# ai4ce/V2X-Sim

Measured on AMD Instinct MI355X. Metric: BEV frames/sec, V2VNet 5-agent detection (256x256 BEV), higher is better.
Workload: dtype bf16

## Files before the change

v2x-sim_amd/csrc/conv_halo.hip:

```cpp
#include "common.h"
#include <cstdlib>

static __device__ __attribute__((aligned(64))) unsigned int g_zero_page_h[16];

typedef const __attribute__((address_space(1))) void *gptr_t;
typedef __attribute__((address_space(3))) void *lptr_t;

__device__ __forceinline__ void glds16h(const void *g, char *lds_wave_base) {
    __builtin_amdgcn_global_load_lds((gptr_t)g, (lptr_t)lds_wave_base, 16, 0, 0);
}

struct HaloArgs {
    const uint16_t *in0;
    const uint16_t *in1;
    const uint32_t *bits;
    int zbits;
    int N, H, W;
    const uint16_t *w;
    const float *scale, *shift;
    int relu;
    void *out;
    int out_cstride, out_coff;
    const uint16_t *w2;
    const float *scale2, *shift2;
// ... 554 lines not shown
    const int fj = lane & 15, fq = lane >> 4;
    char *pb = s_patch + grp * PATCH_BYTES;

    for (int off = wave * 1024; off < W_BYTES; off += 8192)
        glds16h(reinterpret_cast<const char *>(a.w) + off + lane * 16, s_w + off);

    constexpr bool TABLES = (COUT2 == 0);
    constexpr int NP1 = (NS1 + 255) / 256, NP0 = (NS0 + 255) / 256;
    int tb1[TABLES ? NP1 : 1], tb0[NP0 ? NP0 : 1];
#pragma unroll
    for (int t = 0; t < (TABLES ? NP1 : 0); ++t) {
        const int L = wv * 64 + t * 256 + lane;
        const int pix = L / SPP1, phys = L - pix * SPP1;
        const int pr = pix / PW, pc = pix - pr * PW;
        tb1[t] = pix < PH * PW ? (((pr * a.W + pc) * C1 + swz<SPP1>(phys, pc) * 8) | (pr << 20) | (pc << 24)) : -1;
    }
    if constexpr (C0 > 0) {
        constexpr int S0 = SPP0 ? SPP0 : 1;
#pragma unroll
        for (int t = 0; t < NP0; ++t) {
            const int L = wv * 64 + t * 256 + lane;
            const int pix = L / S0, phys = L - pix * S0;
            const int pr = pix / PW0, pc = pix - pr * PW0;
            tb0[t] = pix < PH0 * PW0 ? (((pr * (a.W >> 1) + pc) * C0 + swz<(SPP0 ? SPP0 : 4)>(phys, pc) * 8) | (pr << 20) | (pc << 24)) : -1;
        }
    }

    const int txy = a.tiles_x * a.tiles_y;
    auto coords = [&](int tile, int &n, int &y0, int &x0) {
        n = tile / txy;
        const int r = tile - n * txy;
        const int ty = r / a.tiles_x;
        y0 = ty * TH;
        x0 = (r - ty * a.tiles_x) * TW;
    };
    auto load_patch = [&](int tile) {
        int n, y0, x0;
        coords(tile, n, y0, x0);
        if constexpr (TABLES) {
            const unsigned base = ((unsigned)(n * a.H + y0 - 1) * (unsigned)a.W + (unsigned)(x0 - 1)) * (unsigned)C1;
#pragma unroll
            for (int t = 0; t < NP1; ++t) {
                if (wv * 64 + t * 256 >= NS1) break;
                const int y = y0 - 1 + ((tb1[t] >> 20) & 15), x = x0 - 1 + ((tb1[t] >> 24) & 63);
                const bool ok = tb1[t] >= 0 && (unsigned)y < (unsigned)a.H && (unsigned)x < (unsigned)a.W;
                glds16h(ok ? (const void *)(a.in1 + (base + (unsigned)(tb1[t] & 0xfffff))) : (const void *)g_zero_page_h,
                        pb + NS0 * 16 + (wv * 64 + t * 256) * 16);
            }
        } else {
            for (int base = wv * 64; base < NS1; base += 256) {
                const int L = base + lane;
                const int pix = L / SPP1, phys = L - pix * SPP1;
                const int pr = pix / PW, pc = pix - pr * PW;
                const int y = y0 - 1 + pr, x = x0 - 1 + pc;
                const bool ok = pix < PH * PW && (unsigned)y < (unsigned)a.H && (unsigned)x < (unsigned)a.W;
                const unsigned off = ((unsigned)(n * a.H + y) * (unsigned)a.W + (unsigned)x) * (unsigned)C1 + swz<SPP1>(phys, pc) * 8;
                glds16h(ok ? (const void *)(a.in1 + off) : (const void *)g_zero_page_h, pb + NS0 * 16 + base * 16);
            }
        }
        if constexpr (C0 > 0) {
            const int Hs = a.H >> 1, Ws = a.W >> 1;
            const unsigned base = ((unsigned)(n * Hs + (y0 >> 1) - 1) * (unsigned)Ws + (unsigned)((x0 >> 1) - 1)) * (unsigned)C0;
#pragma unroll
            for (int t = 0; t < NP0; ++t) {
                if (wv * 64 + t * 256 >= NS0) break;
                const int y = (y0 >> 1) - 1 + ((tb0[t] >> 20) & 15), x = (x0 >> 1) - 1 + ((tb0[t] >> 24) & 63);
                const bool ok = tb0[t] >= 0 && (unsigned)y < (unsigned)Hs && (unsigned)x < (unsigned)Ws;
                glds16h(ok ? (const void *)(a.in0 + (base + (unsigned)(tb0[t] & 0xfffff))) : (const void *)g_zero_page_h,
                        pb + (wv * 64 + t * 256) * 16);
            }
        }
    };

    f32x4_t acc[TCO][4];
    constexpr int KC0 = C0 / 32, KC1 = C1 / 32, KC = KC0 + KC1, NG = 3 * KC;
    struct Frags {
        bf16x8_t A[3][TCO];
        bf16x8_t B[8];
    };
    auto load_group = [&](int g, Frags &F) {
        const int kx = g / KC, kk = g - kx * KC;
        if (kk < KC0) {
#pragma unroll
            for (int ky = 0; ky < 3; ++ky) {
                const int kslot = (ky * 3 + kx) * (SPP0 + SPP1) + kk * 4 + fq;
#pragma unroll
                for (int i = 0; i < TCO; ++i)
                    F.A[ky][i] = *reinterpret_cast<const bf16x8_t *>(s_w + (kslot * COUT + i * 16 + fj) * 16);
            }
#pragma unroll
            for (int hr = 0; hr < 3; ++hr)
#pragma unroll
                for (int ch = 0; ch < 2; ++ch) {
                    const int pr = wv + hr;
                    const int pc = ((ch * 16 + fj + kx - 1) >> 1) + 1;
                    F.B[hr * 2 + ch] = *reinterpret_cast<const bf16x8_t *>(pb + ((pr * PW0 + pc) * (SPP0 ? SPP0 : 1) + swz<(SPP0 ? SPP0 : 4)>(kk * 4 + fq, pc)) * 16);
                }
        } else {
            const int kc = kk - KC0;
#pragma unroll
            for (int ky = 0; ky < 3; ++ky) {
                const int kslot = (ky * 3 + kx) * (SPP0 + SPP1) + SPP0 + kc * 4 + fq;
#pragma unroll
                for (int i = 0; i < TCO; ++i)
                    F.A[ky][i] = *reinterpret_cast<const bf16x8_t *>(s_w + (kslot * COUT + i * 16 + fj) * 16);
            }
#pragma unroll
            for (int rr = 0; rr < 4; ++rr)
#pragma unroll
                for (int ch = 0; ch < 2; ++ch) {
                    const int pr = 2 * wv + rr;
                    const int pc = ch * 16 + fj + kx;
                    F.B[rr * 2 + ch] = *reinterpret_cast<const bf16x8_t *>(pb + NS0 * 16 + ((pr * PW + pc) * SPP1 + swz<SPP1>(kc * 4 + fq, pc)) * 16);
                }
        }
    };
    auto mma_group = [&](int g, const Frags &F) {
        const bool half = (g % KC) < KC0;
#pragma unroll
        for (int ky = 0; ky < 3; ++ky)
#pragma unroll
            for (int i = 0; i < TCO; ++i)
#pragma unroll
                for (int f = 0; f < 4; ++f) {
                    const int r = f >> 1, ch = f & 1;
                    const int row = half ? (((r + ky - 1) >> 1) + 1) : (r + ky);
                    acc[i][f] = __builtin_amdgcn_mfma_f32_16x16x32_bf16(F.A[ky][i], F.B[row * 2 + ch], acc[i][f], 0, 0, 0);
                }
    };
    auto compute = [&]() {
#pragma unroll
        for (int i = 0; i < TCO; ++i)
#pragma unroll
            for (int f = 0; f < 4; ++f) acc[i][f] = (f32x4_t){0.f, 0.f, 0.f, 0.f};
        if constexpr (TCO == 2) {
            Frags fr[2];
            load_group(0, fr[0]);
#pragma unroll
            for (int g = 0; g < NG; ++g) {
                if (g + 1 < NG) load_group(g + 1, fr[(g + 1) & 1]);
                __builtin_amdgcn_sched_barrier(0);
                mma_group(g, fr[g & 1]);
                __builtin_amdgcn_sched_barrier(0);
            }
        } else {
            static_assert(C0 == 0 || TCO == 2, "the 64-channel form has one full-resolution source");
            bf16x8_t B[8], A[2][TCO];
            auto load_A = [&](int g, int ky, bf16x8_t (&Ak)[TCO]) {
                const int kx = g / KC, kc = g - kx * KC;
                const int kslot = (ky * 3 + kx) * (SPP0 + SPP1) + SPP0 + kc * 4 + fq;
#pragma unroll
                for (int i = 0; i < TCO; ++i) Ak[i] = *reinterpret_cast<const bf16x8_t *>(s_w + (kslot * COUT + i * 16 + fj) * 16);
            };
#pragma unroll
            for (int g = 0; g < NG; ++g) {
                const int kx = g / KC, kc = g - kx * KC;
#pragma unroll
                for (int rr = 0; rr < 4; ++rr)
#pragma unroll
                    for (int ch = 0; ch < 2; ++ch) {
                        const int pr = 2 * wv + rr, pc = ch * 16 + fj + kx;
                        B[rr * 2 + ch] = *reinterpret_cast<const bf16x8_t *>(pb + NS0 * 16 + ((pr * PW + pc) * SPP1 + swz<SPP1>(kc * 4 + fq, pc)) * 16);
                    }
                load_A(g, 0, A[0]);
#pragma unroll
                for (int ky = 0; ky < 3; ++ky) {
                    if (ky < 2) load_A(g, ky + 1, A[(ky + 1) & 1]);
                    __builtin_amdgcn_sched_barrier(0);
#pragma unroll
                    for (int i = 0; i < TCO; ++i)
#pragma unroll
                        for (int f = 0; f < 4; ++f)
                            acc[i][f] = __builtin_amdgcn_mfma_f32_16x16x32_bf16(A[ky & 1][i], B[((f >> 1) + ky) * 2 + (f & 1)], acc[i][f], 0, 0, 0);
                    __builtin_amdgcn_sched_barrier(0);
                }
            }
        }
    };
    auto epilogue = [&](int tile) {
        int n, y0, x0;
        coords(tile, n, y0, x0);
        int zo = 0;
        asm volatile("" : "+v"(zo));
        const float *ss = s_ss + zo;
        if constexpr (COUT2 > 0) {
            bf16x8_t w2f[TCO2][COUT / 32];
            int w2off = fj * COUT + fq * 8;
            asm volatile("" : "+v"(w2off));
#pragma unroll
            for (int i2 = 0; i2 < TCO2; ++i2)
#pragma unroll
                for (int ks = 0; ks < COUT / 32; ++ks)
                    w2f[i2][ks] = *reinterpret_cast<const bf16x8_t *>(a.w2 + w2off + i2 * 16 * COUT + ks * 32);
            asm volatile("s_waitcnt vmcnt(0)" ::: "memory");
#pragma unroll
            for (int f = 0; f < 4; ++f) {
                bf16x8_t hb[COUT / 32];
#pragma unroll
                for (int ks = 0; ks < COUT / 32; ++ks) {
                    float h[8];
#pragma unroll
                    for (int hf = 0; hf < 2; ++hf) {
                        const int i = 2 * ks + hf;
                        const int kappa = 32 * (i >> 1) + 8 * fq + 4 * (i & 1);
                        const float4 sc = *reinterpret_cast<const float4 *>(ss + kappa);
                        const float4 sf = *reinterpret_cast<const float4 *>(ss + COUT + kappa);
                        h[hf * 4 + 0] = acc[i][f][0] * sc.x + sf.x;
                        h[hf * 4 + 1] = acc[i][f][1] * sc.y + sf.y;
                        h[hf * 4 + 2] = acc[i][f][2] * sc.z + sf.z;
                        h[hf * 4 + 3] = acc[i][f][3] * sc.w + sf.w;
                    }
                    uint4 p;
                    p.x = pack_bf16x2(h[0], h[1]);
                    p.y = pack_bf16x2(h[2], h[3]);
                    p.z = pack_bf16x2(h[4], h[5]);
                    p.w = pack_bf16x2(h[6], h[7]);
                    p.x = v2x_relu_bf16x2_floor(p.x, relu_floor);
                    p.y = v2x_relu_bf16x2_floor(p.y, relu_floor);
                    p.z = v2x_relu_bf16x2_floor(p.z, relu_floor);
                    p.w = v2x_relu_bf16x2_floor(p.w, relu_floor);
                    hb[ks] = __builtin_bit_cast(bf16x8_t, p);
                }
                const int y = y0 + 2 * wv + (f >> 1), x = x0 + (f & 1) * 16 + fj;
                uint16_t *prow = reinterpret_cast<uint16_t *>(a.out) + ((size_t)(n * a.H + y) * a.W + x) * a.out_cstride + a.out_coff;
                if (a.x4) {
                    const uint32_t floor2 = a.relu2 ? 0u : 0x80008000u;
#pragma unroll
                    for (int i2 = 0; i2 + 1 < TCO2; i2 += 2) {
                        uint32_t ox[2], oy[2];
#pragma unroll
                        for (int h = 0; h < 2; ++h) {
                            const int co = (i2 + h) * 16 + fq * 4;
                            const float4 s2 = *reinterpret_cast<const float4 *>(ss + 2 * COUT + co);
                            const float4 t2 = *reinterpret_cast<const float4 *>(ss + 2 * COUT + COUT2 + co);
                            f32x4_t d = (f32x4_t){0.f, 0.f, 0.f, 0.f};
#pragma unroll
                            for (int ks = 0; ks < COUT / 32; ++ks) d = __builtin_amdgcn_mfma_f32_16x16x32_bf16(w2f[i2 + h][ks], hb[ks], d, 0, 0, 0);
                            ox[h] = v2x_relu_bf16x2_floor(pack_bf16x2(d[0] * s2.x + t2.x, d[1] * s2.y + t2.y), floor2);
                            oy[h] = v2x_relu_bf16x2_floor(pack_bf16x2(d[2] * s2.z + t2.z, d[3] * s2.w + t2.w), floor2);
                        }
                        v2x_store_pair_x4(prow + i2 * 16 + fq * 4, fq, ox[0], oy[0], ox[1], oy[1]);
                    }
                    continue;
                }
#pragma unroll
                for (int i2 = 0; i2 < TCO2; ++i2) {
                    const int co = i2 * 16 + fq * 4;
                    const float4 s2 = *reinterpret_cast<const float4 *>(ss + 2 * COUT + co);
                    const float4 t2 = *reinterpret_cast<const float4 *>(ss + 2 * COUT + COUT2 + co);
                    f32x4_t d = (f32x4_t){0.f, 0.f, 0.f, 0.f};
#pragma unroll
                    for (int ks = 0; ks < COUT / 32; ++ks) d = __builtin_amdgcn_mfma_f32_16x16x32_bf16(w2f[i2][ks], hb[ks], d, 0, 0, 0);
                    float v0 = d[0] * s2.x + t2.x, v1 = d[1] * s2.y + t2.y, v2 = d[2] * s2.z + t2.z, v3 = d[3] * s2.w + t2.w;
                    if (a.relu2) {
                        v0 = fmaxf(v0, 0.f);
                        v1 = fmaxf(v1, 0.f);
                        v2 = fmaxf(v2, 0.f);
                        v3 = fmaxf(v3, 0.f);
                    }
                    uint2 o;
                    o.x = pack_bf16x2(v0, v1);
                    o.y = pack_bf16x2(v2, v3);
                    *reinterpret_cast<uint2 *>(prow + co) = o;
                }
            }
            return;
        }
        if (a.x4) {
#pragma unroll
            for (int i = 0; i < TCO; i += 2) {
                float4 sc[2], sf[2];
#pragma unroll
                for (int h = 0; h < 2; ++h) {
                    sc[h] = *reinterpret_cast<const float4 *>(ss + (i + h) * 16 + fq * 4);
                    sf[h] = *reinterpret_cast<const float4 *>(ss + COUT + (i + h) * 16 + fq * 4);
                }
#pragma unroll
                for (int f = 0; f < 4; ++f) {
                    const int y = y0 + 2 * wv + (f >> 1), x = x0 + (f & 1) * 16 + fj;
                    uint32_t ox[2], oy[2];
#pragma unroll
                    for (int h = 0; h < 2; ++h) {
                        ox[h] = v2x_relu_bf16x2_floor(pack_bf16x2(acc[i + h][f][0] * sc[h].x + sf[h].x, acc[i + h][f][1] * sc[h].y + sf[h].y), relu_floor);
                        oy[h] = v2x_relu_bf16x2_floor(pack_bf16x2(acc[i + h][f][2] * sc[h].z + sf[h].z, acc[i + h][f][3] * sc[h].w + sf[h].w), relu_floor);
                    }
                    v2x_store_pair_x4(reinterpret_cast<uint16_t *>(a.out) + ((size_t)(n * a.H + y) * a.W + x) * a.out_cstride + a.out_coff + i * 16 + fq * 4, fq,
                                      ox[0], oy[0], ox[1], oy[1]);
                }
            }
            return;
        }
#pragma unroll
        for (int i = 0; i < TCO; ++i) {
            const int co = i * 16 + fq * 4;
            const float4 sc = *reinterpret_cast<const float4 *>(ss + co);
            const float4 sf = *reinterpret_cast<const float4 *>(ss + COUT + co);
#pragma unroll
            for (int f = 0; f < 4; ++f) {
                const int y = y0 + 2 * wv + (f >> 1), x = x0 + (f & 1) * 16 + fj;
                float v0 = acc[i][f][0] * sc.x + sf.x, v1 = acc[i][f][1] * sc.y + sf.y;
                float v2 = acc[i][f][2] * sc.z + sf.z, v3 = acc[i][f][3] * sc.w + sf.w;
                uint2 o;
                o.x = pack_bf16x2(v0, v1);
                o.y = pack_bf16x2(v2, v3);
                o.x = v2x_relu_bf16x2_floor(o.x, relu_floor);
                o.y = v2x_relu_bf16x2_floor(o.y, relu_floor);
                uint16_t *dst = reinterpret_cast<uint16_t *>(a.out) + ((size_t)(n * a.H + y) * a.W + x) * a.out_cstride + a.out_coff + co;
                *reinterpret_cast<uint2 *>(dst) = o;
            }
        }
    };

    const int n_pairs = a.n_tiles >> 1;
    const v2x_tile_walk walk = v2x_xcd_tile_walk(n_pairs, a.xcd_walk);
    const int K = walk.first < walk.end ? (walk.end - walk.first + walk.step - 1) / walk.step : 0;
    auto tile_of = [&](int k) { return 2 * (walk.first + k * walk.step) + grp; };

    if (grp == 0) load_patch(tile_of(0));
    __syncthreads();

    for (int i = 0; i <= 2 * K; ++i) {
        if ((i & 1) == grp) {
            if ((i >> 1) < K) compute();
        } else {
            const int m = (i - grp - 1) / 2;
            if (m + 1 < K) load_patch(tile_of(m + 1));
            if (m >= 0) {
                epilogue(tile_of(m));
                if constexpr (N_STORES == 8) {
                    if (a.x4) asm volatile("s_waitcnt vmcnt(4)" ::: "memory");
                    else asm volatile("s_waitcnt vmcnt(8)" ::: "memory");
                } else {
                    if (a.x4) asm volatile("s_waitcnt vmcnt(8)" ::: "memory");
                    else asm volatile("s_waitcnt vmcnt(16)" ::: "memory");
                }
            } else {
                asm volatile("s_waitcnt vmcnt(0)" ::: "memory");
            }
        }
        __builtin_amdgcn_sched_barrier(0);
        __builtin_amdgcn_s_barrier();
        __builtin_amdgcn_sched_barrier(0);
    }
    static_assert(N_STORES == 8 || N_STORES == 16, "the counted waits above know 8 or 16 stores per tile and wave");
}

template <int C0, int C1, int COUT, int COUT2 = 0>
static int launch_halo_pp(const HaloArgs &a, hipStream_t s) {
    constexpr int NS1 = round64(PH * PW * (C1 / 8));
    constexpr int NS0 = C0 ? round64(PH0 * PW0 * (C0 / 8)) : 0;
    constexpr int smem = 9 * (C0 + C1) / 8 * COUT * 16 + 2 * (NS0 + NS1) * 16 + 2 * COUT * 4 + 2 * COUT2 * 4;
    static_assert(smem <= 160 * 1024, "LDS budget");
    int grid = 256;
    if (grid > a.n_tiles / 2) grid = a.n_tiles / 2;
    return v2x_launch<conv3x3_halo_pp_kernel<C0, C1, COUT, COUT2>>("conv3x3_halo_pp_kernel", dim3(grid), dim3(512), smem, s, a);
}

constexpr int PWH = PW / 2;

template <int C0, int C1, int COUT>
__global__ __launch_bounds__(512) __attribute__((amdgpu_waves_per_eu(2, 2))) void conv3x3_halo_ppc_kernel(const HaloArgs a) {
    constexpr int SPP0 = C0 / 8, SPP1 = C1 / 8;
    constexpr int NS1 = round64(2 * PH * PWH * SPP1);
    constexpr int NS0 = round64(PH0 * PW0 * SPP0);
    constexpr int PATCH_BYTES = (NS0 + NS1) * 16;
    constexpr int W_UP_BYTES = 16 * SPP0 * COUT * 16;
    constexpr int W_BYTES = W_UP_BYTES + 9 * SPP1 * COUT * 16;
    constexpr int TCO = COUT / 16;
    constexpr int KC0 = C0 / 32, KC1 = C1 / 32;
    static_assert(C0 % 32 == 0 && C1 % 32 == 0 && C0 > 0 && C1 > 0 && TCO == 2, "parity-class form: two sources, 32 output channels");
    static_assert(W_BYTES % 1024 == 0, "weights are moved 1 KiB per wave instruction");
    constexpr int N_STORES = TCO * 4;

    extern __shared__ __attribute__((aligned(16))) char smem[];
    const uint32_t relu_floor = a.relu ? 0u : 0x80008000u;
    char *s_w = smem;
    char *s_patch = smem + W_BYTES;
    float *s_ss = reinterpret_cast<float *>(smem + W_BYTES + 2 * PATCH_BYTES);
    for (int i = threadIdx.x; i < COUT; i += 512) {
        s_ss[i] = a.scale[i];
        s_ss[COUT + i] = a.shift[i];
    }

    const int tid = threadIdx.x;
    const int lane = tid & 63;
    const int wave = __builtin_amdgcn_readfirstlane(tid >> 6);
    const int grp = wave >> 2, wv = wave & 3;
    const int py = wv >> 1, px = wv & 1;
    const int fj = lane & 15, fq = lane >> 4;
    char *pb = s_patch + grp * PATCH_BYTES;

    for (int off = wave * 1024; off < W_BYTES; off += 8192)
        glds16h(reinterpret_cast<const char *>(a.w) + off + lane * 16, s_w + off);

    constexpr int NP1 = (NS1 + 255) / 256, NP0 = (NS0 + 255) / 256;
    int tb1[NP1], tb0[NP0];
#pragma unroll
    for (int t = 0; t < NP1; ++t) {
        const int L = wv * 64 + t * 256 + lane;
        const int pix = L / SPP1, phys = L - pix * SPP1;
        const int q = pix / (PH * PWH), rem = pix - q * (PH * PWH);
        const int pr = rem / PWH, cc = rem - pr * PWH;
        const int pc = 2 * cc + q;
        tb1[t] = pix < 2 * PH * PWH ? (((pr * a.W + pc) * C1 + swz<SPP1>(phys, cc) * 8) | (pr << 20) | (pc << 24)) : -1;
    }
#pragma unroll
    for (int t = 0; t < NP0; ++t) {
        const int L = wv * 64 + t * 256 + lane;
        const int pix = L / SPP0, phys = L - pix * SPP0;
        const int pr = pix / PW0, pc = pix - pr * PW0;
        tb0[t] = pix < PH0 * PW0 ? (((pr * (a.W >> 1) + pc) * C0 + swz<SPP0>(phys, pc) * 8) | (pr << 20) | (pc << 24)) : -1;
    }

    const int txy = a.tiles_x * a.tiles_y;
    auto coords = [&](int tile, int &n, int &y0, int &x0) {
        n = tile / txy;
        const int r = tile - n * txy;
        const int ty = r / a.tiles_x;
        y0 = ty * TH;
        x0 = (r - ty * a.tiles_x) * TW;
    };
    auto load_patch = [&](int tile) {
        int n, y0, x0;
        coords(tile, n, y0, x0);
        {
            const unsigned base = ((unsigned)(n * a.H + y0 - 1) * (unsigned)a.W + (unsigned)(x0 - 1)) * (unsigned)C1;
#pragma unroll
            for (int t = 0; t < NP1; ++t) {
                if (wv * 64 + t * 256 >= NS1) break;
                const int y = y0 - 1 + ((tb1[t] >> 20) & 15), x = x0 - 1 + ((tb1[t] >> 24) & 63);
                const bool ok = tb1[t] >= 0 && (unsigned)y < (unsigned)a.H && (unsigned)x < (unsigned)a.W;
                glds16h(ok ? (const void *)(a.in1 + (base + (unsigned)(tb1[t] & 0xfffff))) : (const void *)g_zero_page_h,
                        pb + NS0 * 16 + (wv * 64 + t * 256) * 16);
            }
        }
        {
            const int Hs = a.H >> 1, Ws = a.W >> 1;
            const unsigned base = ((unsigned)(n * Hs + (y0 >> 1) - 1) * (unsigned)Ws + (unsigned)((x0 >> 1) - 1)) * (unsigned)C0;
#pragma unroll
            for (int t = 0; t < NP0; ++t) {
                if (wv * 64 + t * 256 >= NS0) break;
                const int y = (y0 >> 1) - 1 + ((tb0[t] >> 20) & 15), x = (x0 >> 1) - 1 + ((tb0[t] >> 24) & 63);
                const bool ok = tb0[t] >= 0 && (unsigned)y < (unsigned)Hs && (unsigned)x < (unsigned)Ws;
                glds16h(ok ? (const void *)(a.in0 + (base + (unsigned)(tb0[t] & 0xfffff))) : (const void *)g_zero_page_h,
                        pb + (wv * 64 + t * 256) * 16);
            }
        }
    };

    f32x4_t acc[TCO][4];
    constexpr int NG = 2 * KC0 + 3 * KC1;
    struct Frags {
        bf16x8_t A[3 * TCO];
        bf16x8_t B[9];
    };
    auto load_group = [&](int g, Frags &F) {
        if (g < 2 * KC0) {
            const int kc = g >> 1, b = g & 1;
#pragma unroll
            for (int t = 0; t < 2; ++t)
#pragma unroll
                for (int i = 0; i < TCO; ++i)
                    F.A[t * TCO + i] = *reinterpret_cast<const bf16x8_t *>(s_w + ((((wv * 4 + t * 2 + b) * SPP0 + kc * 4 + fq) * COUT) + i * 16 + fj) * 16);
            const int pc = fj + b + px;
#pragma unroll
            for (int r = 0; r < 5; ++r)
                F.B[r] = *reinterpret_cast<const bf16x8_t *>(pb + (((py + r) * PW0 + pc) * SPP0 + swz<SPP0>(kc * 4 + fq, pc)) * 16);
        } else {
            const int h = g - 2 * KC0, kx = h / KC1, kc = h - kx * KC1;
#pragma unroll
            for (int ky = 0; ky < 3; ++ky)
#pragma unroll
                for (int i = 0; i < TCO; ++i)
                    F.A[ky * TCO + i] = *reinterpret_cast<const bf16x8_t *>(s_w + W_UP_BYTES + ((((ky * 3 + kx) * SPP1 + kc * 4 + fq) * COUT) + i * 16 + fj) * 16);
            const int q = (px + kx) & 1, cc = fj + ((px + kx) >> 1);
#pragma unroll
            for (int r = 0; r < 9; ++r)
                F.B[r] = *reinterpret_cast<const bf16x8_t *>(pb + NS0 * 16 + ((((q * PH) + py + r) * PWH + cc) * SPP1 + swz<SPP1>(kc * 4 + fq, cc)) * 16);
        }
    };
    auto mma_group = [&](int g, const Frags &F) {
// ... 211 lines not shown
```

v2x-sim_amd/csrc/conv_halo_pair.hip:

```cpp
#include "common.h"
#include <cstdlib>

typedef const __attribute__((address_space(1))) void *gptr_p_t;
typedef __attribute__((address_space(3))) void *lptr_p_t;

struct PairArgs {
    const uint32_t *bits;
    int zbits;
    int N, H, W;
    const uint16_t *wA, *wB;
    const float *scA, *shA, *scB, *shB;
    int reluA, reluB;
    uint16_t *out;
    int out_cstride, out_coff;
    int tiles_x, tiles_y, n_tiles;
    int xcd_walk;
    int x4;
};

namespace pair {
constexpr int TH = 8, TW = 32;
constexpr int MH = TH + 2, MW = TW + 2;
constexpr int IH = TH + 4, IW = TW + 4;
constexpr int NMID = MH * MW;
constexpr int NFRAG = (NMID + 15) / 16;
constexpr int FPW = (NFRAG + 3) / 4;
constexpr int W_BYTES = 36 * 32 * 16;
constexpr int IN_PLANE = IH * IW * 16;
constexpr int IN_BYTES = 2 * IN_PLANE;
constexpr int MID_BYTES = NMID * 64;
constexpr int LUT_BYTES = 256 * 16;
#ifndef V2X_PAIR_LDS_PAD_BUILD
#define V2X_PAIR_LDS_PAD_BUILD 0
#endif
constexpr int SMEM = 2 * W_BYTES + IN_BYTES + MID_BYTES + LUT_BYTES + V2X_PAIR_LDS_PAD_BUILD;
#ifndef V2X_HALO_PSWZ_BUILD
#define V2X_HALO_PSWZ_BUILD 1
#endif
__device__ __forceinline__ int swz4(int slot, int x) { return slot ^ ((x >> V2X_HALO_PSWZ_BUILD) & 3); }
typedef short v2x_s16x2_t __attribute__((ext_vector_type(2)));
__device__ __forceinline__ uint32_t relu_bf16x2(uint32_t x) {
    const v2x_s16x2_t r = __builtin_elementwise_max(__builtin_bit_cast(v2x_s16x2_t, x), (v2x_s16x2_t){0, 0});
    return __builtin_bit_cast(uint32_t, r);
}
__device__ __forceinline__ void lds_barrier() {
    asm volatile("s_waitcnt lgkmcnt(0)" ::: "memory");
    __builtin_amdgcn_s_barrier();
    asm volatile("" ::: "memory");
}
}

template <bool X4>
__global__ __launch_bounds__(256) __attribute__((amdgpu_waves_per_eu(2, 2))) void conv3x3_pair_bits_kernel(const PairArgs a) {
    using namespace pair;
    extern __shared__ __attribute__((aligned(16))) char smem[];
    char *s_wA = smem, *s_wB = smem + W_BYTES, *s_in = smem + 2 * W_BYTES, *s_mid = smem + 2 * W_BYTES + IN_BYTES;
    char *s_lut = s_mid + MID_BYTES;

    const int tid = threadIdx.x;
    const int lane = tid & 63;
    const int wave = __builtin_amdgcn_readfirstlane(tid >> 6);
    const int fj = lane & 15, fq = lane >> 4;

    for (int off = wave * 1024; off < W_BYTES; off += 4096) {
        __builtin_amdgcn_global_load_lds((gptr_p_t)(reinterpret_cast<const char *>(a.wA) + off + lane * 16), (lptr_p_t)(s_wA + off), 16, 0, 0);
        __builtin_amdgcn_global_load_lds((gptr_p_t)(reinterpret_cast<const char *>(a.wB) + off + lane * 16), (lptr_p_t)(s_wB + off), 16, 0, 0);
    }

    int in_off[FPW];
    int mid_off[FPW][2];
    int rc[FPW];
#pragma unroll
    for (int t = 0; t < FPW; ++t) {
        const int p = (wave + 4 * t) * 16 + fj;
        const int pc = p < NMID ? p : NMID - 1;
        const int r = pc / MW, c = pc - r * MW;
        in_off[t] = (fq & 1) * IN_PLANE + (r * IW + c) * 16;
        rc[t] = r | (c << 8) | ((p < NMID ? 1 : 0) << 16);
#pragma unroll
        for (int i = 0; i < 2; ++i) mid_off[t][i] = ((r * MW + c) * 4 + swz4(i * 2 + (fq >> 1), c)) * 16 + (fq & 1) * 8;
    }
    int tap_off[5], wA_off[5][2];
#pragma unroll
    for (int st = 0; st < 5; ++st) {
        const int tap = 2 * st + (fq >> 1);
        const int tc = tap < 9 ? tap : 8;
        tap_off[st] = ((tc / 3) * IW + (tc % 3)) * 16;
#pragma unroll
        for (int i = 0; i < 2; ++i)
            wA_off[st][i] = tap < 9 ? ((tap * 4 + (fq & 1)) * 32 + i * 16 + fj) * 16 : 2 * W_BYTES + IN_BYTES + MID_BYTES - 0;
    }
    const uint32_t zmask = (a.zbits >= 16) ? 0xffffu : ((1u << a.zbits) - 1u);
    const int txy = a.tiles_x * a.tiles_y;

    auto fetch_words = [&](int tile, uint32_t (&w)[2], uint32_t &okmask) {
        const int n = tile / txy;
        const int r = tile - n * txy;
        const int ty = r / a.tiles_x, tx = r - ty * a.tiles_x;
        uint32_t m = 0;
#pragma unroll
        for (int s = 0; s < 2; ++s) {
            const int p = min(tid + 256 * s, IH * IW - 1);
            const int pr = p / IW, pcx = p - pr * IW;
            const int y = ty * TH - 2 + pr, x = tx * TW - 2 + pcx;
            const bool ok = (unsigned)y < (unsigned)a.H && (unsigned)x < (unsigned)a.W;
            const int yc = min(max(y, 0), a.H - 1), xc = min(max(x, 0), a.W - 1);
            w[s] = a.bits[(size_t)(n * a.H + yc) * a.W + xc];
            m |= (ok ? 1u : 0u) << s;
        }
        okmask = m;
    };

    float4 scA[2], shA[2], scB[2], shB[2];
#pragma unroll
    for (int i = 0; i < 2; ++i) {
        scA[i] = *reinterpret_cast<const float4 *>(a.scA + i * 16 + fq * 4);
        shA[i] = *reinterpret_cast<const float4 *>(a.shA + i * 16 + fq * 4);
        scB[i] = *reinterpret_cast<const float4 *>(a.scB + i * 16 + fq * 4);
        shB[i] = *reinterpret_cast<const float4 *>(a.shB + i * 16 + fq * 4);
    }

    {
        const uint32_t b = tid, one = 0x3f80u;
        uint4 v;
        v.x = ((b & 1u) ? one : 0u) | ((b & 2u) ? (one << 16) : 0u);
        v.y = ((b & 4u) ? one : 0u) | ((b & 8u) ? (one << 16) : 0u);
        v.z = ((b & 16u) ? one : 0u) | ((b & 32u) ? (one << 16) : 0u);
        v.w = ((b & 64u) ? one : 0u) | ((b & 128u) ? (one << 16) : 0u);
        *reinterpret_cast<uint4 *>(s_lut + tid * 16) = v;
    }
    __syncthreads();
    auto expand_words = [&](const uint32_t (&w)[2], uint32_t okmask) {
#pragma unroll
        for (int s = 0; s < 2; ++s) {
            const int p = tid + 256 * s;
            if (p < IH * IW) {
                const uint32_t word = ((okmask >> s) & 1u) ? (w[s] & zmask) : 0u;
#pragma unroll
                for (int slot = 0; slot < 2; ++slot)
                    *reinterpret_cast<uint4 *>(s_in + slot * IN_PLANE + p * 16) =
                        *reinterpret_cast<const uint4 *>(s_lut + ((word >> (8 * slot)) & 0xffu) * 16);
            }
        }
    };

    const v2x_tile_walk walk = v2x_xcd_tile_walk(a.n_tiles, a.xcd_walk);
    int tile = walk.first;
    uint32_t words[2] = {0u, 0u}, okmask = 0;
    if (tile < walk.end) {
        fetch_words(tile, words, okmask);
        expand_words(words, okmask);
    }
#pragma unroll
    for (int i = 0; i < 2; ++i)
        asm volatile("" ::"v"(scA[i].x), "v"(scA[i].w), "v"(shA[i].x), "v"(shA[i].w), "v"(scB[i].x), "v"(scB[i].w), "v"(shB[i].x), "v"(shB[i].w));
    __syncthreads();

    for (; tile < walk.end; tile += walk.step) {
        const int next = tile + walk.step;
        if (next < walk.end) fetch_words(next, words, okmask);

        const int n = tile / txy;
        const int rr_ = tile - n * txy;
        const int ty = rr_ / a.tiles_x, tx = rr_ - ty * a.tiles_x;

        {
            f32x4_t acc[FPW][2];
#pragma unroll
            for (int t = 0; t < FPW; ++t)
#pragma unroll
                for (int i = 0; i < 2; ++i) acc[t][i] = (f32x4_t){0.f, 0.f, 0.f, 0.f};
#pragma unroll
            for (int st = 0; st < 5; ++st) {
                bf16x8_t A[2], B[FPW];
#pragma unroll
                for (int i = 0; i < 2; ++i) A[i] = *reinterpret_cast<const bf16x8_t *>(smem + wA_off[st][i]);
#pragma unroll
                for (int t = 0; t < FPW; ++t) {
                    B[t] = *reinterpret_cast<const bf16x8_t *>(s_in + in_off[t] + tap_off[st]);
                }
                __builtin_amdgcn_sched_barrier(0);
#pragma unroll
                for (int t = 0; t < FPW; ++t) {
#pragma unroll
                    for (int i = 0; i < 2; ++i) acc[t][i] = __builtin_amdgcn_mfma_f32_16x16x32_bf16(A[i], B[t], acc[t][i], 0, 0, 0);
                }
                __builtin_amdgcn_sched_barrier(0);
            }
#pragma unroll
            for (int t = 0; t < FPW; ++t) {
                const int r = rc[t] & 0xff, c = (rc[t] >> 8) & 0xff;
                const int y = ty * TH - 1 + r, x = tx * TW - 1 + c;
                const bool inside = (unsigned)y < (unsigned)a.H && (unsigned)x < (unsigned)a.W;
                if (!(rc[t] >> 16)) continue;
#pragma unroll
                for (int i = 0; i < 2; ++i) {
                    float v0 = acc[t][i][0] * scA[i].x + shA[i].x, v1 = acc[t][i][1] * scA[i].y + shA[i].y;
                    float v2 = acc[t][i][2] * scA[i].z + shA[i].z, v3 = acc[t][i][3] * scA[i].w + shA[i].w;
                    uint2 o;
                    o.x = pack_bf16x2(v0, v1);
                    o.y = pack_bf16x2(v2, v3);
                    if (a.reluA) {
                        o.x = relu_bf16x2(o.x);
                        o.y = relu_bf16x2(o.y);
                    }
                    o.x = inside ? o.x : 0u;
                    o.y = inside ? o.y : 0u;
                    *reinterpret_cast<uint2 *>(s_mid + mid_off[t][i]) = o;
                }
            }
        }
        lds_barrier();

        {
            f32x4_t acc[2][4];
#pragma unroll
            for (int i = 0; i < 2; ++i)
#pragma unroll
                for (int f = 0; f < 4; ++f) acc[i][f] = (f32x4_t){0.f, 0.f, 0.f, 0.f};
#pragma unroll
            for (int kx = 0; kx < 3; ++kx) {
                bf16x8_t A[3][2], B[8];
#pragma unroll
                for (int ky = 0; ky < 3; ++ky)
#pragma unroll
                    for (int i = 0; i < 2; ++i)
                        A[ky][i] = *reinterpret_cast<const bf16x8_t *>(s_wB + (((ky * 3 + kx) * 4 + fq) * 32 + i * 16 + fj) * 16);
#pragma unroll
                for (int q = 0; q < 4; ++q)
#pragma unroll
                    for (int ch = 0; ch < 2; ++ch) {
                        const int pr = 2 * wave + q, pc = ch * 16 + fj + kx;
                        B[q * 2 + ch] = *reinterpret_cast<const bf16x8_t *>(s_mid + ((pr * MW + pc) * 4 + swz4(fq, pc)) * 16);
                    }
                __builtin_amdgcn_sched_barrier(0);
#pragma unroll
                for (int ky = 0; ky < 3; ++ky)
#pragma unroll
                    for (int i = 0; i < 2; ++i)
#pragma unroll
                        for (int f = 0; f < 4; ++f)
                            acc[i][f] = __builtin_amdgcn_mfma_f32_16x16x32_bf16(A[ky][i], B[((f >> 1) + ky) * 2 + (f & 1)], acc[i][f], 0, 0, 0);
                __builtin_amdgcn_sched_barrier(0);
            }
            if constexpr (X4) {
                const uint32_t floorB = a.reluB ? 0u : 0x80008000u;
#pragma unroll
                for (int f = 0; f < 4; ++f) {
                    const int y = ty * TH + 2 * wave + (f >> 1), x = tx * TW + (f & 1) * 16 + fj;
                    uint32_t ox[2], oy[2];
#pragma unroll
                    for (int h = 0; h < 2; ++h) {
                        ox[h] = v2x_relu_bf16x2_floor(pack_bf16x2(acc[h][f][0] * scB[h].x + shB[h].x, acc[h][f][1] * scB[h].y + shB[h].y), floorB);
                        oy[h] = v2x_relu_bf16x2_floor(pack_bf16x2(acc[h][f][2] * scB[h].z + shB[h].z, acc[h][f][3] * scB[h].w + shB[h].w), floorB);
                    }
                    v2x_store_pair_x4(a.out + ((size_t)(n * a.H + y) * a.W + x) * a.out_cstride + a.out_coff + fq * 4, fq, ox[0], oy[0], ox[1], oy[1]);
                }
            } else {
#pragma unroll
            for (int i = 0; i < 2; ++i) {
                const int co = i * 16 + fq * 4;
                const float4 sc = scB[i], sf = shB[i];
#pragma unroll
                for (int f = 0; f < 4; ++f) {
                    const int y = ty * TH + 2 * wave + (f >> 1), x = tx * TW + (f & 1) * 16 + fj;
                    float v0 = acc[i][f][0] * sc.x + sf.x, v1 = acc[i][f][1] * sc.y + sf.y;
                    float v2 = acc[i][f][2] * sc.z + sf.z, v3 = acc[i][f][3] * sc.w + sf.w;
                    uint2 o;
                    o.x = pack_bf16x2(v0, v1);
                    o.y = pack_bf16x2(v2, v3);
                    if (a.reluB) {
                        o.x = relu_bf16x2(o.x);
                        o.y = relu_bf16x2(o.y);
                    }
                    *reinterpret_cast<uint2 *>(a.out + ((size_t)(n * a.H + y) * a.W + x) * a.out_cstride + a.out_coff + co) = o;
                }
            }
            }
        }
        if (next < a.n_tiles) expand_words(words, okmask);
        lds_barrier();
    }
}


int v2x_conv_tail_dispatch(const v2x_conv_desc *first, const v2x_conv_desc *second, hipStream_t stream);

extern "C" int v2x_conv2d_pair(const v2x_conv_desc *first, const v2x_conv_desc *second, v2x_stream_t stream) {
    V2X_REQUIRE(first && second, "v2x_conv2d_pair: null descriptor");
    if (second->Cout2 > 0 && first->in_format == 0) return v2x_conv_tail_dispatch(first, second, (hipStream_t)stream);
    const v2x_conv_desc *ds[2] = {first, second};
    for (int k = 0; k < 2; ++k) {
        const v2x_conv_desc *d = ds[k];
        V2X_REQUIRE(d->ksize == 3 && d->stride == 1 && d->pad == 1 && d->w_layout == 1 && d->C0 == 32 && d->C1 == 0 &&
                        d->Cout == 32 && d->Cout2 == 0 && d->epilogue == V2X_EPI_BF16 && d->up0 == 0 && d->split == 0,
                    "v2x_conv2d_pair: layer %d must be a halo-packed 3x3 stride-1 32 -> 32 bf16 layer", k);
        V2X_REQUIRE(d->weight && d->scale && d->shift, "v2x_conv2d_pair: layer %d has null parameters", k);
    }
    V2X_REQUIRE(first->in_format == 1 && first->in0 && first->in_zbits >= 1 && first->in_zbits <= 16,
                "v2x_conv2d_pair: the first layer reads the voxelizer's bit grid (1 <= zbits <= 16)");
    V2X_REQUIRE(second->out && second->out_cstride >= 32 + second->out_coff && second->out_cstride % 4 == 0 && second->out_coff % 4 == 0,
                "v2x_conv2d_pair: bad output view");
    V2X_REQUIRE(first->N == second->N && first->H == second->H && first->W == second->W, "v2x_conv2d_pair: extents differ");
    V2X_REQUIRE(first->N >= 0 && first->H > 0 && first->W > 0 && first->H % pair::TH == 0 && first->W % pair::TW == 0,
                "v2x_conv2d_pair: H %% 8 == 0 and W %% 32 == 0 required (H=%d W=%d)", first->H, first->W);
    V2X_REQUIRE((long long)first->N * first->H * first->W < (1ll << 31), "v2x_conv2d_pair: N*H*W must fit 31 bits");
    if (first->N == 0) return V2X_OK;
    PairArgs a;
    a.xcd_walk = v2x_tune(V2X_TUNE_HALO_XCD);
    a.x4 = v2x_x4_ok(second->out, second->out_cstride, second->out_coff, 32);
    a.bits = reinterpret_cast<const uint32_t *>(first->in0);
    a.zbits = first->in_zbits;
    a.N = first->N;
    a.H = first->H;
    a.W = first->W;
    a.wA = first->weight;
    a.wB = second->weight;
    a.scA = first->scale;
    a.shA = first->shift;
    a.scB = second->scale;
    a.shB = second->shift;
    a.reluA = first->relu;
    a.reluB = second->relu;
    a.out = reinterpret_cast<uint16_t *>(second->out);
    a.out_cstride = second->out_cstride;
    a.out_coff = second->out_coff;
    a.tiles_x = a.W / pair::TW;
    a.tiles_y = a.H / pair::TH;
    a.n_tiles = a.N * a.tiles_x * a.tiles_y;
    int grid = v2x_num_cus() * 2;
    if (grid > a.n_tiles) grid = a.n_tiles;
    if (a.x4) return v2x_launch<conv3x3_pair_bits_kernel<true>>("conv3x3_pair_bits_kernel", dim3(grid), dim3(256), pair::SMEM, (hipStream_t)stream, a);
    return v2x_launch<conv3x3_pair_bits_kernel<false>>("conv3x3_pair_bits_kernel", dim3(grid), dim3(256), pair::SMEM, (hipStream_t)stream, a);
}
```

Before: 6646.

## Software-pipeline LDS fragment reads with MFMA and overlap patch prefetch with epilogue

```diff
diff --git a/v2x-sim_amd/csrc/conv_halo.hip b/v2x-sim_amd/csrc/conv_halo.hip
--- a/v2x-sim_amd/csrc/conv_halo.hip
+++ b/v2x-sim_amd/csrc/conv_halo.hip
@@ -730,32 +730,49 @@
 #pragma unroll
                 for (int i = 0; i < TCO; ++i) Ak[i] = *reinterpret_cast<const bf16x8_t *>(s_w + (kslot * COUT + i * 16 + fj) * 16);
             };
-#pragma unroll
-            for (int g = 0; g < NG; ++g) {
+            auto load_B2 = [&](int g, int r0) {
                 const int kx = g / KC, kc = g - kx * KC;
 #pragma unroll
-                for (int rr = 0; rr < 4; ++rr)
+                for (int rr = r0; rr < r0 + 2; ++rr)
 #pragma unroll
                     for (int ch = 0; ch < 2; ++ch) {
                         const int pr = 2 * wv + rr, pc = ch * 16 + fj + kx;
                         B[rr * 2 + ch] = *reinterpret_cast<const bf16x8_t *>(pb + NS0 * 16 + ((pr * PW + pc) * SPP1 + swz<SPP1>(kc * 4 + fq, pc)) * 16);
                     }
-                load_A(g, 0, A[0]);
+            };
+            load_B2(0, 0);
+            load_A(0, 0, A[0]);
+#pragma unroll
+            for (int g = 0; g < NG; ++g) {
 #pragma unroll
                 for (int ky = 0; ky < 3; ++ky) {
-                    if (ky < 2) load_A(g, ky + 1, A[(ky + 1) & 1]);
+                    const int s = (3 * g + ky) & 1;
                     __builtin_amdgcn_sched_barrier(0);
 #pragma unroll
-                    for (int i = 0; i < TCO; ++i)
+                    for (int f = 0; f < 4; ++f)
+                        acc[0][f] = __builtin_amdgcn_mfma_f32_16x16x32_bf16(A[s][0], B[((f >> 1) + ky) * 2 + (f & 1)], acc[0][f], 0, 0, 0);
+                    __builtin_amdgcn_sched_barrier(0);
+                    if (ky == 0) {
+                        load_B2(g, 2);
+                        load_A(g, 1, A[s ^ 1]);
+                    } else if (ky == 1) {
+                        load_A(g, 2, A[s ^ 1]);
+                    } else if (g + 1 < NG) {
+                        load_B2(g + 1, 0);
+                        load_A(g + 1, 0, A[s ^ 1]);
+                    }
+                    __builtin_amdgcn_sched_barrier(0);
+#pragma unroll
+                    for (int i = 1; i < TCO; ++i)
 #pragma unroll
                         for (int f = 0; f < 4; ++f)
-                            acc[i][f] = __builtin_amdgcn_mfma_f32_16x16x32_bf16(A[ky & 1][i], B[((f >> 1) + ky) * 2 + (f & 1)], acc[i][f], 0, 0, 0);
+                            acc[i][f] = __builtin_amdgcn_mfma_f32_16x16x32_bf16(A[s][i], B[((f >> 1) + ky) * 2 + (f & 1)], acc[i][f], 0, 0, 0);
                     __builtin_amdgcn_sched_barrier(0);
                 }
             }
         }
     };
-    auto epilogue = [&](int tile) {
+    auto epilogue = [&](int tile, int next) {
         int n, y0, x0;
         coords(tile, n, y0, x0);
         int zo = 0;
@@ -770,7 +787,22 @@
 #pragma unroll
                 for (int ks = 0; ks < COUT / 32; ++ks)
                     w2f[i2][ks] = *reinterpret_cast<const bf16x8_t *>(a.w2 + w2off + i2 * 16 * COUT + ks * 32);
-            asm volatile("s_waitcnt vmcnt(0)" ::: "memory");
+            __builtin_amdgcn_sched_barrier(0);
+            float4 sc1[TCO], sf1[TCO], s2v[TCO2], t2v[TCO2];
+#pragma unroll
+            for (int i = 0; i < TCO; ++i) {
+                const int kappa = 32 * (i >> 1) + 8 * fq + 4 * (i & 1);
+                sc1[i] = *reinterpret_cast<const float4 *>(ss + kappa);
+                sf1[i] = *reinterpret_cast<const float4 *>(ss + COUT + kappa);
+            }
+#pragma unroll
+            for (int i2 = 0; i2 < TCO2; ++i2) {
+                s2v[i2] = *reinterpret_cast<const float4 *>(ss + 2 * COUT + i2 * 16 + fq * 4);
+                t2v[i2] = *reinterpret_cast<const float4 *>(ss + 2 * COUT + COUT2 + i2 * 16 + fq * 4);
+            }
+            __builtin_amdgcn_sched_barrier(0);
+            if (next >= 0) load_patch(next);
+            __builtin_amdgcn_sched_barrier(0);
 #pragma unroll
             for (int f = 0; f < 4; ++f) {
                 bf16x8_t hb[COUT / 32];
@@ -780,9 +812,7 @@
 #pragma unroll
                     for (int hf = 0; hf < 2; ++hf) {
                         const int i = 2 * ks + hf;
-                        const int kappa = 32 * (i >> 1) + 8 * fq + 4 * (i & 1);
-                        const float4 sc = *reinterpret_cast<const float4 *>(ss + kappa);
-                        const float4 sf = *reinterpret_cast<const float4 *>(ss + COUT + kappa);
+                        const float4 sc = sc1[i], sf = sf1[i];
                         h[hf * 4 + 0] = acc[i][f][0] * sc.x + sf.x;
                         h[hf * 4 + 1] = acc[i][f][1] * sc.y + sf.y;
                         h[hf * 4 + 2] = acc[i][f][2] * sc.z + sf.z;
@@ -808,9 +838,7 @@
                         uint32_t ox[2], oy[2];
 #pragma unroll
                         for (int h = 0; h < 2; ++h) {
-                            const int co = (i2 + h) * 16 + fq * 4;
-                            const float4 s2 = *reinterpret_cast<const float4 *>(ss + 2 * COUT + co);
-                            const float4 t2 = *reinterpret_cast<const float4 *>(ss + 2 * COUT + COUT2 + co);
+                            const float4 s2 = s2v[i2 + h], t2 = t2v[i2 + h];
                             f32x4_t d = (f32x4_t){0.f, 0.f, 0.f, 0.f};
 #pragma unroll
                             for (int ks = 0; ks < COUT / 32; ++ks) d = __builtin_amdgcn_mfma_f32_16x16x32_bf16(w2f[i2 + h][ks], hb[ks], d, 0, 0, 0);
@@ -824,8 +852,7 @@
 #pragma unroll
                 for (int i2 = 0; i2 < TCO2; ++i2) {
                     const int co = i2 * 16 + fq * 4;
-                    const float4 s2 = *reinterpret_cast<const float4 *>(ss + 2 * COUT + co);
-                    const float4 t2 = *reinterpret_cast<const float4 *>(ss + 2 * COUT + COUT2 + co);
+                    const float4 s2 = s2v[i2], t2 = t2v[i2];
                     f32x4_t d = (f32x4_t){0.f, 0.f, 0.f, 0.f};
 #pragma unroll
                     for (int ks = 0; ks < COUT / 32; ++ks) d = __builtin_amdgcn_mfma_f32_16x16x32_bf16(w2f[i2][ks], hb[ks], d, 0, 0, 0);
@@ -844,23 +871,26 @@
             }
             return;
         }
+        float4 sc[TCO], sf[TCO];
+#pragma unroll
+        for (int i = 0; i < TCO; ++i) {
+            sc[i] = *reinterpret_cast<const float4 *>(ss + i * 16 + fq * 4);
+            sf[i] = *reinterpret_cast<const float4 *>(ss + COUT + i * 16 + fq * 4);
+        }
+        __builtin_amdgcn_sched_barrier(0);
+        if (next >= 0) load_patch(next);
+        __builtin_amdgcn_sched_barrier(0);
         if (a.x4) {
 #pragma unroll
             for (int i = 0; i < TCO; i += 2) {
-                float4 sc[2], sf[2];
-#pragma unroll
-                for (int h = 0; h < 2; ++h) {
-                    sc[h] = *reinterpret_cast<const float4 *>(ss + (i + h) * 16 + fq * 4);
-                    sf[h] = *reinterpret_cast<const float4 *>(ss + COUT + (i + h) * 16 + fq * 4);
-                }
 #pragma unroll
                 for (int f = 0; f < 4; ++f) {
                     const int y = y0 + 2 * wv + (f >> 1), x = x0 + (f & 1) * 16 + fj;
                     uint32_t ox[2], oy[2];
 #pragma unroll
                     for (int h = 0; h < 2; ++h) {
-                        ox[h] = v2x_relu_bf16x2_floor(pack_bf16x2(acc[i + h][f][0] * sc[h].x + sf[h].x, acc[i + h][f][1] * sc[h].y + sf[h].y), relu_floor);
-                        oy[h] = v2x_relu_bf16x2_floor(pack_bf16x2(acc[i + h][f][2] * sc[h].z + sf[h].z, acc[i + h][f][3] * sc[h].w + sf[h].w), relu_floor);
+                        ox[h] = v2x_relu_bf16x2_floor(pack_bf16x2(acc[i + h][f][0] * sc[i + h].x + sf[i + h].x, acc[i + h][f][1] * sc[i + h].y + sf[i + h].y), relu_floor);
+                        oy[h] = v2x_relu_bf16x2_floor(pack_bf16x2(acc[i + h][f][2] * sc[i + h].z + sf[i + h].z, acc[i + h][f][3] * sc[i + h].w + sf[i + h].w), relu_floor);
                     }
                     v2x_store_pair_x4(reinterpret_cast<uint16_t *>(a.out) + ((size_t)(n * a.H + y) * a.W + x) * a.out_cstride + a.out_coff + i * 16 + fq * 4, fq,
                                       ox[0], oy[0], ox[1], oy[1]);
@@ -871,13 +901,11 @@
 #pragma unroll
         for (int i = 0; i < TCO; ++i) {
             const int co = i * 16 + fq * 4;
-            const float4 sc = *reinterpret_cast<const float4 *>(ss + co);
-            const float4 sf = *reinterpret_cast<const float4 *>(ss + COUT + co);
 #pragma unroll
             for (int f = 0; f < 4; ++f) {
                 const int y = y0 + 2 * wv + (f >> 1), x = x0 + (f & 1) * 16 + fj;
-                float v0 = acc[i][f][0] * sc.x + sf.x, v1 = acc[i][f][1] * sc.y + sf.y;
-                float v2 = acc[i][f][2] * sc.z + sf.z, v3 = acc[i][f][3] * sc.w + sf.w;
+                float v0 = acc[i][f][0] * sc[i].x + sf[i].x, v1 = acc[i][f][1] * sc[i].y + sf[i].y;
+                float v2 = acc[i][f][2] * sc[i].z + sf[i].z, v3 = acc[i][f][3] * sc[i].w + sf[i].w;
                 uint2 o;
                 o.x = pack_bf16x2(v0, v1);
                 o.y = pack_bf16x2(v2, v3);
@@ -902,9 +930,9 @@
             if ((i >> 1) < K) compute();
         } else {
             const int m = (i - grp - 1) / 2;
-            if (m + 1 < K) load_patch(tile_of(m + 1));
+            if (m + 1 < K && m < 0) load_patch(tile_of(m + 1));
             if (m >= 0) {
-                epilogue(tile_of(m));
+                epilogue(tile_of(m), m + 1 < K ? tile_of(m + 1) : -1);
                 if constexpr (N_STORES == 8) {
                     if (a.x4) asm volatile("s_waitcnt vmcnt(4)" ::: "memory");
                     else asm volatile("s_waitcnt vmcnt(8)" ::: "memory");
diff --git a/v2x-sim_amd/csrc/conv_halo_pair.hip b/v2x-sim_amd/csrc/conv_halo_pair.hip
--- a/v2x-sim_amd/csrc/conv_halo_pair.hip
+++ b/v2x-sim_amd/csrc/conv_halo_pair.hip
@@ -170,21 +170,45 @@
             for (int t = 0; t < FPW; ++t)
 #pragma unroll
                 for (int i = 0; i < 2; ++i) acc[t][i] = (f32x4_t){0.f, 0.f, 0.f, 0.f};
+            bf16x8_t A[2][2], B[2][FPW];
+            auto read_A = [&](int st, bf16x8_t (&Ak)[2]) {
+#pragma unroll
+                for (int i = 0; i < 2; ++i) Ak[i] = *reinterpret_cast<const bf16x8_t *>(smem + wA_off[st][i]);
+            };
+            auto read_B = [&](int st, int t0, bf16x8_t (&Bk)[FPW]) {
+#pragma unroll
+                for (int t = t0; t < t0 + 2; ++t) Bk[t] = *reinterpret_cast<const bf16x8_t *>(s_in + in_off[t] + tap_off[st]);
+            };
+            auto mma = [&](int p, int t0, int t1) {
+#pragma unroll
+                for (int t = t0; t < t1; ++t)
+#pragma unroll
+                    for (int i = 0; i < 2; ++i) acc[t][i] = __builtin_amdgcn_mfma_f32_16x16x32_bf16(A[p][i], B[p][t], acc[t][i], 0, 0, 0);
+            };
+            static_assert(FPW == 6, "the read schedule below is written for six fragments per wave");
+            read_A(0, A[0]);
+#pragma unroll
+            for (int t = 0; t < FPW; t += 2) read_B(0, t, B[0]);
 #pragma unroll
             for (int st = 0; st < 5; ++st) {
-                bf16x8_t A[2], B[FPW];
-#pragma unroll
-                for (int i = 0; i < 2; ++i) A[i] = *reinterpret_cast<const bf16x8_t *>(smem + wA_off[st][i]);
-#pragma unroll
-                for (int t = 0; t < FPW; ++t) {
-                    B[t] = *reinterpret_cast<const bf16x8_t *>(s_in + in_off[t] + tap_off[st]);
-                }
-                __builtin_amdgcn_sched_barrier(0);
-#pragma unroll
-                for (int t = 0; t < FPW; ++t) {
-#pragma unroll
-                    for (int i = 0; i < 2; ++i) acc[t][i] = __builtin_amdgcn_mfma_f32_16x16x32_bf16(A[i], B[t], acc[t][i], 0, 0, 0);
-                }
+                const int p = st & 1;
+                __builtin_amdgcn_sched_barrier(0);
+                mma(p, 0, 2);
+                __builtin_amdgcn_sched_barrier(0);
+                if (st < 4) {
+                    read_A(st + 1, A[p ^ 1]);
+                    read_B(st + 1, 0, B[p ^ 1]);
+                }
+                __builtin_amdgcn_sched_barrier(0);
+                mma(p, 2, 4);
+                __builtin_amdgcn_sched_barrier(0);
+                if (st < 4) read_B(st + 1, 2, B[p ^ 1]);
+                __builtin_amdgcn_sched_barrier(0);
+                mma(p, 4, 5);
+                __builtin_amdgcn_sched_barrier(0);
+                if (st < 4) read_B(st + 1, 4, B[p ^ 1]);
+                __builtin_amdgcn_sched_barrier(0);
+                mma(p, 5, 6);
                 __builtin_amdgcn_sched_barrier(0);
             }
 #pragma unroll
@@ -210,38 +234,55 @@
                 }
             }
         }
+        bf16x8_t A[3][2], B[8];
+        auto read_wB = [&](int kx, int ky) {
+#pragma unroll
+            for (int i = 0; i < 2; ++i) A[ky][i] = *reinterpret_cast<const bf16x8_t *>(s_wB + (((ky * 3 + kx) * 4 + fq) * 32 + i * 16 + fj) * 16);
+        };
+        auto read_mid = [&](int kx, int q0) {
+#pragma unroll
+            for (int q = q0; q < q0 + 2; ++q)
+#pragma unroll
+                for (int ch = 0; ch < 2; ++ch) {
+                    const int pr = 2 * wave + q, pc = ch * 16 + fj + kx;
+                    B[q * 2 + ch] = *reinterpret_cast<const bf16x8_t *>(s_mid + ((pr * MW + pc) * 4 + swz4(fq, pc)) * 16);
+                }
+        };
         lds_barrier();
-
         {
             f32x4_t acc[2][4];
 #pragma unroll
             for (int i = 0; i < 2; ++i)
 #pragma unroll
                 for (int f = 0; f < 4; ++f) acc[i][f] = (f32x4_t){0.f, 0.f, 0.f, 0.f};
+            read_mid(0, 0);
+            read_wB(0, 0);
 #pragma unroll
             for (int kx = 0; kx < 3; ++kx) {
-                bf16x8_t A[3][2], B[8];
-#pragma unroll
-                for (int ky = 0; ky < 3; ++ky)
+#pragma unroll
+                for (int ky = 0; ky < 3; ++ky) {
+                    __builtin_amdgcn_sched_barrier(0);
+#pragma unroll
+                    for (int f = 0; f < 2; ++f)
+                        acc[0][f] = __builtin_amdgcn_mfma_f32_16x16x32_bf16(A[ky][0], B[((f >> 1) + ky) * 2 + (f & 1)], acc[0][f], 0, 0, 0);
+                    __builtin_amdgcn_sched_barrier(0);
+                    if (ky == 0) {
+                        read_mid(kx, 2);
+                        read_wB(kx, 1);
+                    } else if (ky == 1) {
+                        read_wB(kx, 2);
+                    } else if (kx < 2) {
+                        read_mid(kx + 1, 0);
+                        read_wB(kx + 1, 0);
+                    }
+                    __builtin_amdgcn_sched_barrier(0);
 #pragma unroll
                     for (int i = 0; i < 2; ++i)
-                        A[ky][i] = *reinterpret_cast<const bf16x8_t *>(s_wB + (((ky * 3 + kx) * 4 + fq) * 32 + i * 16 + fj) * 16);
-#pragma unroll
-                for (int q = 0; q < 4; ++q)
-#pragma unroll
-                    for (int ch = 0; ch < 2; ++ch) {
-                        const int pr = 2 * wave + q, pc = ch * 16 + fj + kx;
-                        B[q * 2 + ch] = *reinterpret_cast<const bf16x8_t *>(s_mid + ((pr * MW + pc) * 4 + swz4(fq, pc)) * 16);
-                    }
-                __builtin_amdgcn_sched_barrier(0);
-#pragma unroll
-                for (int ky = 0; ky < 3; ++ky)
-#pragma unroll
-                    for (int i = 0; i < 2; ++i)
-#pragma unroll
-                        for (int f = 0; f < 4; ++f)
+#pragma unroll
+                        for (int f = (i == 0 ? 2 : 0); f < 4; ++f)
                             acc[i][f] = __builtin_amdgcn_mfma_f32_16x16x32_bf16(A[ky][i], B[((f >> 1) + ky) * 2 + (f & 1)], acc[i][f], 0, 0, 0);
-                __builtin_amdgcn_sched_barrier(0);
+                    __builtin_amdgcn_sched_barrier(0);
+                }
             }
             if constexpr (X4) {
                 const uint32_t floorB = a.reluB ? 0u : 0x80008000u;
```

Result: no change. 6690 (median of 6 runs) (+0.7%).
